# RazonIn4K/image-restoration-platform

Hardware: AMD Instinct MI355X
Metric: restored images/sec @1024x1024 bs=8 (higher is better)
Workload: dtype bf16; 1 GPU; 1024x1024 RGB u8, batch 8 per GPU: fused classifier scan + RestoreNet-v0 (43 convs, 779.9 GFLOP/image), seeded random-init weights; global_batch=8, parallelism=per-image data parallel x1, no collective, streams=1

## Files before the change

image_restoration_platform_amd/csrc/conv_down.hip:

```cpp
#include "conv_mfma.hpp"
#include "persist.hpp"

namespace ire {

namespace {

typedef __bf16 bf16x8_t __attribute__((ext_vector_type(8)));
typedef __bf16 bf16x2_t __attribute__((ext_vector_type(2)));
typedef float f32x2_t __attribute__((ext_vector_type(2)));
typedef float f32x16_t __attribute__((ext_vector_type(16)));
typedef unsigned u32x4_t __attribute__((ext_vector_type(4)));

#ifndef DN_LD_NT
#define DN_LD_NT 0
#endif
constexpr int DN_THREADS = 512;
constexpr int DN_TH = 16, DN_TW = 32;
constexpr int DN_IH = DN_TH + 1, DN_IW = DN_TW + 1;
constexpr int DN_IN_CHUNKS = DN_IH * DN_IW * 4;
constexpr int DN_IN_ITERS = (DN_IN_CHUNKS + DN_THREADS - 1) / DN_THREADS;
constexpr int DN_IN_BYTES = DN_IN_ITERS * DN_THREADS * 16;
constexpr int DN_NT = 64, DN_NTL = 2;
constexpr int DN_W_BYTES_MAX = 4 * 4 * DN_NT * 16;
constexpr int DN_W_BASE = 2 * DN_IN_BYTES;
constexpr int DN_MAIN = DN_W_BASE + 3 * DN_W_BYTES_MAX;
constexpr int DN_RED_HALF = 8 * (DN_NT / 8) * 4 * 4;
constexpr int DN_LDS = DN_MAIN + 2 * DN_RED_HALF + 256 * 4;
static_assert(DN_LDS <= 160 * 1024, "LDS");

__device__ __forceinline__ unsigned dn_pack(float a, float b) {
    f32x2_t f = {a, b};
    return __builtin_bit_cast(unsigned, __builtin_convertvector(f, bf16x2_t));
}
__device__ __forceinline__ void dn_glds16(const void* gsrc, unsigned lds_dst_uniform) {
    unsigned keep;
    asm volatile("s_mov_b32 %0, m0\n\ts_mov_b32 m0, %2\n\ts_nop 0\n\tglobal_load_lds_dwordx4 %1, off\n\ts_mov_b32 m0, %0"
                 : "=&s"(keep) : "v"(gsrc), "s"(lds_dst_uniform) : "memory");
}
template <int N> __device__ __forceinline__ float dn_ror_add(float v) {
    const int r = __builtin_amdgcn_update_dpp(0, __builtin_bit_cast(int, v), 0x120 + N, 0xf, 0xf, false);
    return v + __builtin_bit_cast(float, r);
}
__device__ __forceinline__ float dn_swap16_add(float v) {
    float x = v, y = v;
    asm volatile("v_nop\n\tv_nop\n\tv_permlane16_swap_b32 %0, %1" : "+v"(x), "+v"(y));
    return x + y;
}

__host__ __device__ constexpr int dn_ntaps(int p) { return ((p >> 1) ? 2 : 1) * ((p & 1) ? 2 : 1); }
__host__ __device__ constexpr int dn_slab_off(int p) { return p == 0 ? 0 : p == 1 ? 4096 : p == 2 ? 12288 : 20480; }
constexpr int DN_GROUP_BYTES = 9 * 4 * DN_NT * 16;

struct DnRegs { u32x4_t v[DN_IN_ITERS]; };
__host__ __device__ constexpr int dn_dma_iters(int p) { return (dn_ntaps(p) * 4 * DN_NT + DN_THREADS - 1) / DN_THREADS; }
template <int N> __device__ __forceinline__ void dn_wait_vm(bool counted) {
    if (counted) asm volatile("s_waitcnt vmcnt(%0)" :: "n"(N) : "memory");
    else asm volatile("s_waitcnt vmcnt(0)" ::: "memory");
}

__global__ __launch_bounds__(DN_THREADS) void conv_down_kernel(ConvArgs a) {
    __shared__ __attribute__((aligned(16))) unsigned char smem[DN_LDS];
    const unsigned smem_lds = (unsigned)(size_t)(__attribute__((address_space(3))) unsigned char*)smem;
    const int tid = threadIdx.x;
    const int lane = tid & 63, wave = tid >> 6;
    const int r = lane & 31, h = lane >> 5;
    const int c8_fixed = tid & 3;

    const int tiles_per_img = a.tiles_x * a.tiles_y;
    const int nkc = a.nkc;
    PersistCursor cursor(a.tiles_x, a.tiles_y, a.nimg, a.nblocks, 4 * nkc, (int)gridDim.x, (int)blockIdx.x, a.walk_rev != 0);
    const int my_items = cursor.my_items;
    const int S = cursor.S;
    if (S == 0) return;
    using StageInfo = PersistStage;
    StageInfo sq0 = cursor.cur, sq1 = cursor.next(), sq2 = cursor.next();

    const int Cin = a.cin0;
    const int cin_shift = 31 - __builtin_clz(Cin);

    int a_off[2][4];
#pragma unroll
    for (int m = 0; m < 2; ++m)
#pragma unroll
        for (int o = 0; o < 4; ++o) {
            const int dy = (o >> 1) - 1, dx = (o & 1) - 1;
            const int p = (wave * 2 + m + 1 + dy) * DN_IW + r + 1 + dx;
            a_off[m][o] = (p * 4 + (h ^ ((p >> 2) & 3))) * 16;
        }
    const int b_off = (h * DN_NT + r) * 16;

    unsigned coff[DN_IN_ITERS], cokb = 0;
    auto item_offsets = [&](const PersistItem& it) {
        const int y0 = 2 * (it.ty * DN_TH - 1), x0 = 2 * (it.tx * DN_TW - 1);
        int t2 = tid;
// ... 66 lines not shown
            const int gg = (st_nb * DN_NT) / Gs + tid;
            float* st = a.stats + (((size_t)st_img * tiles_per_img + st_tile) * 8 + gg) * 2;
            st[0] = s; st[1] = q;
        }
        st_img = -1;
    };
    auto init_acc = [&](int nb) {
        const float* bl = bias_lds + nb * DN_NT + 8 * h;
#pragma unroll
        for (int j = 0; j < DN_NTL; ++j)
#pragma unroll
            for (int q = 0; q < 4; ++q) {
                const float4 bv = *reinterpret_cast<const float4*>(bl + j * 32 + 16 * (q >> 1) + 4 * (q & 1));
#pragma unroll
                for (int m = 0; m < 2; ++m) { acc[m][j][4 * q + 0] = bv.x; acc[m][j][4 * q + 1] = bv.y; acc[m][j][4 * q + 2] = bv.z; acc[m][j][4 * q + 3] = bv.w; }
            }
    };
    auto epilogue = [&](const PersistItem& it) __attribute__((always_inline)) {
        int r_e = r, h_e = h, w_e = wave;
        asm volatile("" : "+v"(r_e), "+v"(h_e), "+v"(w_e));
        char* obase = reinterpret_cast<char*>(a.out) + (size_t)it.img * a.Hout * a.Wout * a.cout * 2;
        const __amdgpu_buffer_rsrc_t orsrc = __builtin_amdgcn_make_buffer_rsrc(obase, 0, a.Hout * a.Wout * a.cout * 2, 0x00020000);
        const bf16x2_t ones = __builtin_bit_cast(bf16x2_t, 0x3f803f80u);
        float* redw = red_base + red_par * (DN_RED_HALF / 4);
        const int ox = it.tx * DN_TW + r_e;
        bool inb[2];
        unsigned offs[2];
#pragma unroll
        for (int m = 0; m < 2; ++m) {
            const int oy = it.ty * DN_TH + w_e * 2 + m;
            inb[m] = oy < a.Hout && ox < a.Wout;
            offs[m] = ((unsigned)((oy * a.Wout + ox) * a.cout + it.nb * DN_NT) << 1) + (unsigned)(h_e * 16);
        }
#pragma unroll
        for (int j = 0; j < DN_NTL; ++j)
#pragma unroll
            for (int pp = 0; pp < 2; ++pp) {
                float sA = 0.f, qA = 0.f;
#pragma unroll
                for (int m = 0; m < 2; ++m) {
                    const f32x16_t& c = acc[m][j];
                    const unsigned w[4] = {dn_pack(c[8 * pp + 0], c[8 * pp + 1]), dn_pack(c[8 * pp + 2], c[8 * pp + 3]),
                                           dn_pack(c[8 * pp + 4], c[8 * pp + 5]), dn_pack(c[8 * pp + 6], c[8 * pp + 7])};
                    float ts = 0.f, tq = 0.f;
#pragma unroll
                    for (int d = 0; d < 4; ++d) {
                        const bf16x2_t wv = __builtin_bit_cast(bf16x2_t, w[d]);
                        ts = __builtin_amdgcn_fdot2_f32_bf16(wv, ones, ts, false);
                        tq = __builtin_amdgcn_fdot2_f32_bf16(wv, wv, tq, false);
                    }
                    sA += inb[m] ? ts : 0.f; qA += inb[m] ? tq : 0.f;
                    const u32x4_t wv4 = {w[0], w[1], w[2], w[3]};
                    __builtin_amdgcn_raw_buffer_store_b128(wv4, orsrc, inb[m] ? offs[m] + (unsigned)(j * 64 + pp * 32) : 0xffffffffu, 0, IRE_ST_PART);
                }
                sA = dn_ror_add<1>(sA); qA = dn_ror_add<1>(qA);
                sA = dn_ror_add<2>(sA); qA = dn_ror_add<2>(qA);
                sA = dn_ror_add<4>(sA); qA = dn_ror_add<4>(qA);
                sA = dn_ror_add<8>(sA); qA = dn_ror_add<8>(qA);
                sA = dn_swap16_add(sA); qA = dn_swap16_add(qA);
                if ((lane & 31) == 0) {
                    float* d = redw + (wave * 8 + j * 4 + 2 * pp + h_e) * 4;
                    d[0] = sA; d[1] = qA; d[2] = 0.f; d[3] = 0.f;
                }
            }
#pragma unroll
        for (int m = 0; m < 2; ++m)
#pragma unroll
            for (int j = 0; j < DN_NTL; ++j) asm volatile("" : "=v"(acc[m][j]));
        st_img = it.img; st_tile = it.tile; st_nb = it.nb; st_par = red_par; red_par ^= 1;
    };

    DnRegs R0, R1;
    int widx = 0;
    bool warm = false;
    auto stage = [&](auto phase_tag, auto last_tag) {
        constexpr int PHASE = decltype(phase_tag)::value, PAR = PHASE & 1;
        constexpr bool LAST = decltype(last_tag)::value;
        constexpr int PA = PHASE >> 1, PB = PHASE & 1, NTY = PA ? 2 : 1, NTX = PB ? 2 : 1, NTAPS = NTY * NTX;
        constexpr int D1 = dn_dma_iters((PHASE + 1) & 3), D2 = dn_dma_iters((PHASE + 2) & 3);
        const unsigned char* ib = smem + PAR * DN_IN_BYTES;
        uint4* in_nxt = reinterpret_cast<uint4*>(smem + (PAR ^ 1) * DN_IN_BYTES);
        const unsigned char* wb = smem + DN_W_BASE + widx * DN_W_BYTES_MAX + b_off;
        const int w2 = widx == 0 ? 2 : widx - 1;
        DnRegs& Rn = PAR ? R0 : R1;
        DnRegs& Rf = PAR ? R1 : R0;
        load_stage(sq2, Rf);
        {
            constexpr int NPH = (PHASE + 2) & 3;
            constexpr int pieces = dn_ntaps(NPH) * 4 * DN_NT;
            const unsigned char* ws = wslab(sq2);
            const int wave_u = __builtin_amdgcn_readfirstlane(wave);
            const unsigned w_dst_lds = smem_lds + (unsigned)(DN_W_BASE + w2 * DN_W_BYTES_MAX);
#pragma unroll
            for (int i = 0; i < D2; ++i) {
                int cbase = i * DN_THREADS + wave_u * 64;
                if ((i + 1) * DN_THREADS > pieces) cbase = cbase % pieces;
                dn_glds16(ws + (size_t)(cbase + lane) * 16, w_dst_lds + cbase * 16);
// ... 47 lines not shown
        for (int i = 0; i < DN_IN_ITERS; ++i) asm volatile("" : "+v"(R0.v[i]));
        const uint4* ws0 = reinterpret_cast<const uint4*>(wslab(sq0));
        const uint4* ws1 = reinterpret_cast<const uint4*>(wslab(sq1));
        uint4* wd = reinterpret_cast<uint4*>(smem + DN_W_BASE);
        for (int i = tid; i < dn_ntaps(0) * 4 * DN_NT; i += DN_THREADS) wd[i] = ws0[i];
        for (int i = tid; i < dn_ntaps(1) * 4 * DN_NT; i += DN_THREADS) wd[DN_W_BYTES_MAX / 16 + i] = ws1[i];
        uint4* in0 = reinterpret_cast<uint4*>(smem);
#pragma unroll
        for (int i = 0; i < DN_IN_ITERS; ++i) store_chunk(i, R0, in0);
        load_stage(sq1, R1);
    }
    __syncthreads();
    for (int k = 0; k < my_items; ++k) {
        init_acc(sq0.it.nb);
        for (int kc = 0; kc + 1 < nkc; ++kc) {
            stage(std::integral_constant<int, 0>{}, std::false_type{}); stage(std::integral_constant<int, 1>{}, std::false_type{});
            stage(std::integral_constant<int, 2>{}, std::false_type{}); stage(std::integral_constant<int, 3>{}, std::false_type{});
        }
        stage(std::integral_constant<int, 0>{}, std::false_type{}); stage(std::integral_constant<int, 1>{}, std::false_type{});
        stage(std::integral_constant<int, 2>{}, std::false_type{}); stage(std::integral_constant<int, 3>{}, std::true_type{});
    }
    asm volatile("s_waitcnt vmcnt(0)" ::: "memory");
    __syncthreads();
    flush_stats();
}

}

void conv_down_launch(const ConvArgs& a, hipStream_t stream) {
    if (a.cout % 64 || a.cout > 256 || a.nkc < 1 || a.stats == nullptr) fail(IRE_ERR_INTERNAL, "internal: conv_down shape");
    const int items = a.tiles_x * a.tiles_y * a.nimg * a.nblocks;
    const int cus = persistent_grid_cus();
    const int grid = items < cus ? items : cus;
    hipLaunchKernelGGL(conv_down_kernel, dim3(grid), dim3(DN_THREADS), 0, stream, a);
    IRE_HIP(hipGetLastError());
}

}
```

image_restoration_platform_amd/csrc/conv_mfma.hpp:

```cpp
#pragma once
#include "common.hpp"
#include "conv_kind.hpp"

#ifndef IRE_ST_LINE
#define IRE_ST_LINE 16
#endif
#ifndef IRE_LD_ONCE
#define IRE_LD_ONCE 2
#endif
#ifndef IRE_LD_IN
#define IRE_LD_IN 0
#endif
#ifndef IRE_ST_PART
#define IRE_ST_PART 0
#endif

#include <cstdlib>

namespace ire {

inline int persistent_grid_cus() {
    static const int forced = [] { const char* v = std::getenv("IRE_GRID_CUS"); return v ? std::atoi(v) : 0; }();
    int dev = 0, cus = 256;
    (void)hipGetDevice(&dev);
// ... 7 lines not shown
    const void* in0;
    const void* in1;
    int cin0, cin1;
    int kc_split;
    int nkc;
    const unsigned short* w;
    const unsigned short* w1;
    const float* bias;
    const float2* ab;
    const float* gn_stats;
    int gn_parts, gn_hw;
    const float* gn_gamma;
    const float* gn_beta;
    const float* gn_film;
    int gn_film_stride, gn_film_off;
    float2* ab_w;
    const unsigned short* resid;
    unsigned short* out;
    const unsigned char* u8_in;
    unsigned char* u8_out;
    float* stats;
    int Hin, Win, Hout, Wout, cout;
    int tiles_x, tiles_y, nimg, nblocks;
    int group_size;
    int prio_young;
    int in_rows;
    int in_row_off;
    int iy_lo, iy_span;
    int fp8;
    const float* oscale;
    int w4_nt;
    const void* zeros;
    unsigned long long* stamps;
    int walk_rev;
};

void conv_launch(ConvKind kind, const ConvArgs& a, hipStream_t stream);

void conv_rb_launch(bool resid, bool fused_act, const ConvArgs& a, hipStream_t stream);
void conv_w4_launch(bool resid, const ConvArgs& a, hipStream_t stream);
void conv_f8_launch(bool resid, const ConvArgs& a, hipStream_t stream);
void conv_stem_launch(const ConvArgs& a, hipStream_t stream);
void conv_down_launch(const ConvArgs& a, hipStream_t stream);
void conv_head_launch(const ConvArgs& a, hipStream_t stream);
void conv_pc_launch(bool resid, bool head, const ConvArgs& a, hipStream_t stream);
void conv_pk_launch(bool resid, const ConvArgs& a, hipStream_t stream);
void conv_up_subpixel_launch(const ConvArgs& a, hipStream_t stream);
void conv_upq_launch(const ConvArgs& a, hipStream_t stream);
void conv_dnq_launch(const ConvArgs& a, hipStream_t stream);
void conv_up_launch(const ConvArgs& a, hipStream_t stream);

}
```

image_restoration_platform_amd/csrc/conv_stem.hip:

```cpp
#include "conv_mfma.hpp"
#include "persist.hpp"

#include <type_traits>

namespace ire {

namespace {

typedef __bf16 bf16x8_t __attribute__((ext_vector_type(8)));
typedef __bf16 bf16x2_t __attribute__((ext_vector_type(2)));
typedef float f32x2_t __attribute__((ext_vector_type(2)));
typedef float f32x16_t __attribute__((ext_vector_type(16)));
typedef unsigned u32x4_t __attribute__((ext_vector_type(4)));

constexpr int ST_THREADS = 512, ST_TH = 16, ST_TW = 32, ST_IH = ST_TH + 2, ST_IW = ST_TW + 2;
constexpr int ST_RB = ST_IW * 3;
constexpr int ST_PW = ST_IW + 2;
constexpr int ST_ROW = ST_PW * 4;
constexpr int ST_ITERS = (ST_IH * ST_RB + ST_THREADS - 1) / ST_THREADS;

__device__ __forceinline__ unsigned st_pack(float a, float b) {
    f32x2_t f = {a, b};
    return __builtin_bit_cast(unsigned, __builtin_convertvector(f, bf16x2_t));
}
template <int N> __device__ __forceinline__ float st_ror_add(float v) {
    const int r = __builtin_amdgcn_update_dpp(0, __builtin_bit_cast(int, v), 0x120 + N, 0xf, 0xf, false);
    return v + __builtin_bit_cast(float, r);
}
__device__ __forceinline__ float st_swap16_add(float v) {
    float x = v, y = v;
    asm volatile("v_nop\n\tv_nop\n\tv_permlane16_swap_b32 %0, %1" : "+v"(x), "+v"(y));
    return x + y;
}

__global__ __launch_bounds__(ST_THREADS) void conv_stem_kernel(ConvArgs a) {
    __shared__ __attribute__((aligned(16))) unsigned short tile[2][ST_IH * ST_ROW];
    __shared__ float red[2][8][8][2];
    const int tid = threadIdx.x, lane = tid & 63, wave = tid >> 6, r = lane & 31, h = lane >> 5;

    const u32x4_t* wf = reinterpret_cast<const u32x4_t*>(a.w);
    const bf16x8_t w0 = __builtin_bit_cast(bf16x8_t, wf[(0 * 2 + h) * 32 + r]);
    const bf16x8_t w1 = __builtin_bit_cast(bf16x8_t, wf[(1 * 2 + h) * 32 + r]);
    const bf16x8_t w2 = __builtin_bit_cast(bf16x8_t, wf[(2 * 2 + h) * 32 + r]);
    f32x16_t bias_acc;
#pragma unroll
    for (int i = 0; i < 16; ++i) bias_acc[i] = a.bias[16 * (i >> 3) + 8 * h + (i & 7)];
    const int foff = (2 * wave * ST_PW + r + 2 * h) * 4;
    for (int i = tid; i < 2 * ST_IH * ST_ROW / 2; i += ST_THREADS) reinterpret_cast<unsigned*>(&tile[0][0])[i] = 0u;
    __syncthreads();
    int spy[ST_ITERS], sb[ST_ITERS], spx[ST_ITERS], srel[ST_ITERS];
#pragma unroll
    for (int it = 0; it < ST_ITERS; ++it) {
        const int i = tid + it * ST_THREADS;
        spy[it] = i / ST_RB; sb[it] = i - spy[it] * ST_RB;
        spx[it] = sb[it] / 3;
        srel[it] = (spy[it] * a.Win + spx[it]) * 3 + (sb[it] - spx[it] * 3);
    }

    const int tiles_per_img = a.tiles_x * a.tiles_y;
    const unsigned char* in = reinterpret_cast<const unsigned char*>(a.in0);
    const bf16x2_t ones = __builtin_bit_cast(bf16x2_t, 0x3f803f80u);
    unsigned pv[ST_ITERS];
    auto request = [&](const PersistItem& ri) {
        const int iy0 = ri.ty * ST_TH - 1, ix0 = ri.tx * ST_TW - 1;
        const long long base = (((long long)ri.img * a.in_rows + iy0 + a.in_row_off) * a.Win + ix0) * 3;
#pragma unroll
        for (int it = 0; it < ST_ITERS; ++it) {
            const bool ok = spy[it] < ST_IH && (unsigned)(iy0 + spy[it] - a.iy_lo) < (unsigned)a.iy_span && (unsigned)(ix0 + spx[it]) < (unsigned)a.Win;
            const unsigned v = in[ok ? base + srel[it] : 0];
            pv[it] = ok ? v : 0u;
        }
    };
    int par = 0;
    PersistCursor cursor(a.tiles_x, a.tiles_y, a.nimg, 1, 1, (int)gridDim.x, (int)blockIdx.x, a.walk_rev != 0);
    const int n_items = cursor.my_items;
    PersistItem nx = cursor.cur.it;
    if (n_items > 0) request(nx);
    for (int k = 0; k < n_items; ++k) {
        const int img = nx.img, t = nx.tile, ty = nx.ty, tx = nx.tx;
        unsigned short* tl = tile[par];
#pragma unroll
        for (int it = 0; it < ST_ITERS; ++it)
            if (spy[it] < ST_IH) tl[spy[it] * ST_ROW + spx[it] * 4 + (sb[it] - spx[it] * 3)] = (unsigned short)(__builtin_bit_cast(unsigned, (float)pv[it]) >> 16);
        if (k + 1 < n_items) { nx = cursor.next().it; request(nx); }
        __syncthreads();
        const int ox = tx * ST_TW + r;
        char* obase = reinterpret_cast<char*>(a.out) + (size_t)img * a.Hout * a.Wout * 64;
        float gs[2][2] = {{0.f, 0.f}, {0.f, 0.f}}, gq[2][2] = {{0.f, 0.f}, {0.f, 0.f}};
#pragma unroll
        for (int m = 0; m < 2; ++m) {
            u32x4_t f[3];
#pragma unroll
            for (int ky = 0; ky < 3; ++ky) {
                const uint2* fp = reinterpret_cast<const uint2*>(tl + foff + (m + ky) * ST_ROW);
                const uint2 lo = fp[0], hi = fp[1];
                f[ky] = u32x4_t{lo.x, lo.y, hi.x, hi.y};
            }
            f32x16_t c = __builtin_amdgcn_mfma_f32_32x32x16_bf16(w0, __builtin_bit_cast(bf16x8_t, f[0]), bias_acc, 0, 0, 0);
            c = __builtin_amdgcn_mfma_f32_32x32x16_bf16(w1, __builtin_bit_cast(bf16x8_t, f[1]), c, 0, 0, 0);
            c = __builtin_amdgcn_mfma_f32_32x32x16_bf16(w2, __builtin_bit_cast(bf16x8_t, f[2]), c, 0, 0, 0);
            const int oy = ty * ST_TH + 2 * wave + m;
            const bool inb = ox < a.Wout && oy < a.Hout;
            const float mf = inb ? 1.f : 0.f;
#pragma unroll
            for (int pp = 0; pp < 2; ++pp) {
                const unsigned w[4] = {st_pack(c[8 * pp + 0], c[8 * pp + 1]), st_pack(c[8 * pp + 2], c[8 * pp + 3]),
                                       st_pack(c[8 * pp + 4], c[8 * pp + 5]), st_pack(c[8 * pp + 6], c[8 * pp + 7])};
#pragma unroll
                for (int d = 0; d < 4; ++d) {
                    const bf16x2_t wv = __builtin_bit_cast(bf16x2_t, w[d]);
                    const float s1 = __builtin_amdgcn_fdot2_f32_bf16(wv, ones, 0.f, false), q1 = __builtin_amdgcn_fdot2_f32_bf16(wv, wv, 0.f, false);
                    gs[pp][d >> 1] = __builtin_fmaf(s1, mf, gs[pp][d >> 1]);
                    gq[pp][d >> 1] = __builtin_fmaf(q1, mf, gq[pp][d >> 1]);
                }
                if (inb) {
                    const u32x4_t wv4 = {w[0], w[1], w[2], w[3]};
                    *reinterpret_cast<u32x4_t*>(obase + ((size_t)oy * a.Wout + ox) * 64 + (16 * pp + 8 * h) * 2) = wv4;
                }
            }
            __builtin_amdgcn_sched_barrier(0);
        }
        if (a.stats) {
            const bool b0 = lane & 1, b1 = lane & 2;
            auto xch = [&](float keep, float give, auto ctrl_tag) __attribute__((always_inline)) -> float {
                const int gg = __builtin_amdgcn_update_dpp(0, __builtin_bit_cast(int, give), decltype(ctrl_tag)::value, 0xf, 0xf, false);
                return keep + __builtin_bit_cast(float, gg);
            };
            const float vs[4] = {gs[0][0], gs[0][1], gs[1][0], gs[1][1]}, vq[4] = {gq[0][0], gq[0][1], gq[1][0], gq[1][1]};
            float u[4], t2[2];
#pragma unroll
            for (int k = 0; k < 4; ++k) u[k] = xch(b0 ? vq[k] : vs[k], b0 ? vs[k] : vq[k], std::integral_constant<int, 0xb1>{});
#pragma unroll
            for (int k = 0; k < 2; ++k) t2[k] = xch(b1 ? u[2 + k] : u[k], b1 ? u[k] : u[2 + k], std::integral_constant<int, 0x4e>{});
            t2[0] = st_ror_add<4>(t2[0]); t2[1] = st_ror_add<4>(t2[1]);
            t2[0] = st_ror_add<8>(t2[0]); t2[1] = st_ror_add<8>(t2[1]);
            t2[0] = st_swap16_add(t2[0]); t2[1] = st_swap16_add(t2[1]);
            if ((lane & 28) == 0) {
                const int g0 = 4 * (b1 ? 1 : 0) + 2 * h;
                red[par][wave][g0][b0 ? 1 : 0] = t2[0];
                red[par][wave][g0 + 1][b0 ? 1 : 0] = t2[1];
            }
            __syncthreads();
            if (tid < 8) {
                float s = 0.f, q = 0.f;
#pragma unroll
                for (int w = 0; w < 8; ++w) { s += red[par][w][tid][0]; q += red[par][w][tid][1]; }
                float* st = a.stats + (((size_t)img * tiles_per_img + t) * 8 + tid) * 2;
                st[0] = s; st[1] = q;
            }
        }
        par ^= 1;
    }
}

}

void conv_stem_launch(const ConvArgs& a, hipStream_t stream) {
    if (a.cout != 32 || a.Hout != a.Hin || a.Wout != a.Win || !a.stats) fail(IRE_ERR_INTERNAL, "internal: conv_stem shape");
    const int items = a.tiles_x * a.tiles_y * a.nimg;
    const int cus = persistent_grid_cus();
    const int grid = items < 2 * cus ? items : 2 * cus;
    hipLaunchKernelGGL(conv_stem_kernel, dim3(grid), dim3(ST_THREADS), 0, stream, a);
    IRE_HIP(hipGetLastError());
}

}
```

image_restoration_platform_amd/csrc/engine.cpp:

```cpp
#include "engine.hpp"
#include "encode.hpp"
#include "deflate.hpp"
#include "jpeg.hpp"
#include "jpeg_dec.hpp"

#include <chrono>
#include <cmath>
#include <cstdlib>
#include <cstring>
#include <fstream>

#include "gn.hpp"
#include "strips.hpp"
#include "weight_pack.hpp"
#include "grey_tables.inc"

namespace ire {

namespace {

inline double now_s() {
    return std::chrono::duration<double>(std::chrono::steady_clock::now().time_since_epoch()).count();
}

}

Engine::Engine(const ire_config& cfg) {
    int ndev = 0;
    hipError_t e = hipGetDeviceCount(&ndev);
    if (e != hipSuccess || ndev <= 0)
        fail(IRE_ERR_UNAVAILABLE, "service unavailable: no HIP device visible (the engine has no CPU fallback)");
    device_ = cfg.device_index;
    if (device_ < 0 || device_ >= ndev) fail(IRE_ERR_INVALID_INPUT, "invalid device_index");
    IRE_HIP(hipSetDevice(device_));
    hipDeviceProp_t prop;
    IRE_HIP(hipGetDeviceProperties(&prop, device_));
    if (std::strncmp(prop.gcnArchName, "gfx950", 6) != 0)
        fail(IRE_ERR_UNAVAILABLE, std::string("service unavailable: device is ") + prop.gcnArchName +
                                      ", this engine is built for gfx950 (MI355X) only");
    if (cfg.precision != IRE_PRECISION_BF16 && cfg.precision != IRE_PRECISION_FP8) fail(IRE_ERR_INVALID_INPUT, "invalid precision");
    precision_ = cfg.precision;
    max_batch_ = cfg.max_batch > 0 ? cfg.max_batch : 8;
    if (max_batch_ > 64) fail(IRE_ERR_INVALID_INPUT, "invalid max_batch (1..64)");
    num_lanes_ = cfg.num_streams > 0 ? cfg.num_streams : 1;
    if (num_lanes_ > 16) num_lanes_ = 16;
    constexpr uint32_t kResultBits = IRE_FLAG_RESULT_PNG_BASE64 | IRE_FLAG_RESULT_PNG_DEFLATE | IRE_FLAG_RESULT_JPEG;
    if (cfg.flags & ~(kResultBits | IRE_FLAG_DECODE_PROGRESSIVE)) fail(IRE_ERR_INVALID_INPUT, "invalid ire_config.flags (unknown bits set)");
    if (((cfg.flags & kResultBits) & ((cfg.flags & kResultBits) - 1)) != 0) fail(IRE_ERR_INVALID_INPUT, "invalid ire_config.flags (two result formats set)");
    flags_ = cfg.flags;
    sw_ = ConvSwitches::from_env();
    cus_ = persistent_grid_cus();
    if (const char* v = std::getenv("IRE_SNAKE")) snake_ = std::atoi(v) != 0;
    if (const char* v = std::getenv("IRE_JPEG_DEC_TIMES")) dec_times_ = std::atoi(v) != 0;
    if (const char* v = std::getenv("IRE_JPEG_DEC_WINDOWS")) dec_min_windows_ = (uint32_t)std::max(0, std::atoi(v));
    if (const char* v = std::getenv("IRE_RB_STAMPS")) {
        stamps_cout_ = std::atoi(v);
        stamps_resid_ = std::strchr(v, 'r') != nullptr;
    }
    if (const char* v = std::getenv("IRE_W4_TL")) stamps_tl_ = v;

    IRE_HIP(hipStreamCreateWithFlags(&main_stream_, hipStreamNonBlocking));
    for (auto& ev : ev_) IRE_HIP(hipEventCreate(&ev));
    IRE_HIP(hipEventCreateWithFlags(&fork_ev_, hipEventDisableTiming));
    IRE_HIP(hipEventCreateWithFlags(&busy_ev_, hipEventDisableTiming));
    lanes_.resize(num_lanes_);
    for (auto& L : lanes_) {
        IRE_HIP(hipStreamCreateWithFlags(&L.stream, hipStreamNonBlocking));
        IRE_HIP(hipEventCreateWithFlags(&L.done, hipEventDisableTiming));
    }

    unsigned int* d_lin = tables_mem_.alloc<unsigned int>(sizeof(kLin16));
    unsigned int* d_thr = tables_mem_.alloc<unsigned int>(sizeof(kGreyThr));
    unsigned char* d_inv = tables_mem_.alloc<unsigned char>(5008);
    IRE_HIP(hipMemset(d_inv, 0, 5008));
    IRE_HIP(hipMemcpy(d_lin, kLin16, sizeof(kLin16), hipMemcpyHostToDevice));
    IRE_HIP(hipMemcpy(d_thr, kGreyThr, sizeof(kGreyThr), hipMemcpyHostToDevice));
    IRE_HIP(hipMemcpy(d_inv, kGreyInv, sizeof(kGreyInv), hipMemcpyHostToDevice));
    tables_ = ClassifierTables{d_lin, d_thr, d_inv};
    if (stamps_cout_) {
        stamps_dev_.grow(8 * 2 * 64 * 10 * 8);
        IRE_HIP(hipMemset(stamps_dev_.get<void>(), 0, 8 * 2 * 64 * 10 * 8));
    }

    if (cfg.weights_path && cfg.weights_path[0]) load_weights_file(cfg.weights_path);
}
// ... 636 lines not shown
    const ConvDesc& d = cw.desc;
    ConvSite site;
    site.lin = op.lin; site.lout = op.lout; site.use_ab = op.use_ab; site.has_in1 = op.in1 != BUF_NONE; site.stats_out = op.stats_out;
    site.nimg = g.nimg; site.h = g.h; site.w = g.w; site.H = g.H; site.halo = g.halo; site.has_up = g.has_up; site.has_down = g.has_down;
    site.y0 = g.y0; site.cus = cus_;
    const ConvPlan p = plan_conv(sw_, d, site, precision_ == IRE_PRECISION_FP8);

    auto in_ptr = [&](int id) -> const unsigned short* { return id == BUF_NONE ? nullptr : g.buf[id >> 3][id & 7]; };
    auto out_ptr = [&](int id) -> unsigned short* {
        if (id == BUF_NONE) return nullptr;
        const int l = id >> 3;
        return g.buf[l][id & 7] + (size_t)g.halo * (g.w >> l) * kWidths[l];
    };
    const int Hout = g.h >> op.lout, Wout = g.w >> op.lout;
    ConvArgs a{};
    a.in0 = (d.kind == CONV_STEM) ? (const void*)g.img_in : (const void*)in_ptr(op.in0);
    a.in1 = in_ptr(op.in1);
    if (p.in1_first_row) a.in1 = in_ptr(op.in1) + (size_t)g.halo * Wout * d.cout;
    a.cin0 = d.cin0; a.cin1 = p.cin1; a.kc_split = d.kc_split; a.nkc = p.nkc; a.nblocks = p.nblocks; a.w4_nt = p.w4_nt; a.fp8 = p.fp8;
    const unsigned short* const slabs[] = {nullptr, cw.d_w, cw.d_wp, cw.d_w4, cw.d_w4h, cw.d_wstem, cw.d_wd, cw.d_wu, cw.d_wuf, cw.d_wdq, cw.d_wuq, cw.d_wsq,
                                           cw.d_wsk, reinterpret_cast<const unsigned short*>(cw.d_w8x), reinterpret_cast<const unsigned short*>(cw.d_w8)};
    const float* const biases[] = {cw.d_bias, cw.d_bias_uf, cw.d_bias8};
    a.w = slabs[p.w]; a.w1 = slabs[p.w1]; a.bias = biases[p.bias];
    if (p.fp8) a.oscale = cw.d_oscale;
    if (p.zeros) a.zeros = d_zero_.get<void>();
    a.ab = op.use_ab ? R.ab : nullptr; a.resid = out_ptr(op.resid); a.out = out_ptr(op.out);
    a.u8_in = d.kind == CONV_HEAD ? g.img_in + (size_t)g.halo * g.w * 3 : nullptr;
    a.u8_out = d.kind == CONV_HEAD ? g.img_out : nullptr;
    a.Hin = g.h >> op.lin; a.Win = g.w >> op.lin; a.Hout = Hout; a.Wout = Wout;
    a.in_rows = p.in_rows; a.in_row_off = p.in_row_off; a.iy_lo = p.iy_lo; a.iy_span = p.iy_span;
    a.cout = p.cout; a.group_size = p.group_size; a.tiles_x = p.tiles_x; a.tiles_y = p.tiles_y; a.nimg = g.nimg;
    if (op.stats_out) a.stats = (R.stats_alt ? R.stats_alt : R.stats) + p.stats_offset();
    a.prio_young = sw_.prio_young;
    a.walk_rev = R.snake && R.next_rev && p.kernel != K_V1;
    R.next_rev = !a.walk_rev;
    const bool rb = d.kind == CONV_RB1 || d.kind == CONV_RB2;
    if (stamps_dev_ && rb && d.cout == stamps_cout_ && (d.kind == CONV_RB2) == stamps_resid_ && (!stamps_taken_ || !stamps_tl_.empty() || std::getenv("IRE_STAMPS_RAW"))) {
        a.stamps = stamps_dev_.get<unsigned long long>();
        stamps_taken_ = true;
    }
    if (R.gn_pending) {
        if (p.folds_gn) {
            const GNW& gn = *R.gn_pending;
            a.gn_stats = R.gn_stats; a.gn_parts = R.gn_parts; a.gn_hw = (g.H >> gn.level) * (g.w >> gn.level);
            a.gn_gamma = gn.d_gamma; a.gn_beta = gn.d_beta; a.gn_film = R.film; a.gn_film_stride = kFilmDim; a.gn_film_off = kFilmOff[gn.level];
            a.ab_w = R.ab;
            R.gn_pending = nullptr;
        } else flush_gn(R, g);
    }
    prof_begin(p.fam, R.stream, p.flops, p.bytes);
    switch (p.kernel) {
        case K_V1: conv_launch(d.kind, a, R.stream); break;
        case K_F8: conv_f8_launch(p.resid, a, R.stream); break;
        case K_PK: conv_pk_launch(p.resid, a, R.stream); break;
        case K_W4: conv_w4_launch(p.resid, a, R.stream); break;
        case K_PC: conv_pc_launch(p.resid, false, a, R.stream); break;
        case K_RB: conv_rb_launch(p.resid, p.fused_act, a, R.stream); break;
        case K_PC_HEAD: conv_pc_launch(false, true, a, R.stream); break;
        case K_RB_HEAD: conv_head_launch(a, R.stream); break;
        case K_DNQ: conv_dnq_launch(a, R.stream); break;
        case K_DOWN: conv_down_launch(a, R.stream); break;
        case K_STEM: conv_stem_launch(a, R.stream); break;
        case K_UPQ: conv_upq_launch(a, R.stream); break;
        case K_UP_FUSED:
        case K_UP_SUB: conv_up_subpixel_launch(a, R.stream); break;
        case K_UP_RB: conv_up_launch(a, R.stream); break;
    }
    prof_tag(p.key, p.kname, op.lout, d.cin, d.cout, p.flops_exec);
    prof_end(R.stream);
    if (op.stats_out) {
        R.stat_parts = p.stat_parts;
        if (R.stats_alt) std::swap(R.stats, R.stats_alt);
    }
    if (capture_ && !op.name.empty() && a.out && g.halo == 0) capture(op.name.c_str(), a.out, (size_t)g.nimg * Hout * Wout * d.cout, R.stream);
    if (capture_ && !op.name.empty() && a.out && g.halo == 1)
        capture_rows(op.name.c_str(), a.out, (size_t)Hout * Wout * d.cout, (size_t)(g.H >> op.lout) * Wout * d.cout,
                     (size_t)(g.y0 >> op.lout) * Wout * d.cout, R.stream);
    if (capture_ && a.ab != nullptr && g.halo == 0)
        capture_f32(((op.name.empty() ? std::string("head") : op.name) + ".ab").c_str(), reinterpret_cast<const float*>(R.ab), (size_t)g.nimg * d.cin * 2, R.stream);
}

void Engine::flush_gn(Run& R, const Geo& g) {
    const GNW& gn = *R.gn_pending;
    prof_begin(FAM_GN, R.stream, 0, 0);
    gn_finalize_launch(R.gn_stats, g.nimg, R.gn_parts, gn.C, (g.H >> gn.level) * (g.w >> gn.level), gn.d_gamma, gn.d_beta, R.film, kFilmDim,
                       kFilmOff[gn.level], R.ab, R.stream);
    prof_end(R.stream);
    R.gn_pending = nullptr;
}

void Engine::exec_op(Run& R, const Op& op, const Geo& g) {
    switch (op.kind) {
        case Op::GN: {
            R.gn_pending = op.gn; R.gn_stats = R.stats; R.gn_parts = R.stat_parts;
            if (!sw_.gn_fold || g.halo) flush_gn(R, g);
            break;
        }
        case Op::CONV: exec_conv(R, op, g); break;
    }
}

void Engine::run_network(Lane& L, int nimg, int h, int w, const uint8_t* d_in, uint8_t* d_out, const float* d_film) {
    Run R;
    R.stream = L.stream; R.stats = L.v.stats; R.stats_alt = L.v.stats2; R.ab = L.v.ab; R.film = d_film;
    R.snake = snake_;
    const Geo g = geo_of_lane(L, nimg, h, w, d_in, d_out);
    prof_chain_ = false;
    prof_chainable_ = capture_ == false;
    prof_skip_ = prof_on_ == 2 && prof_every_ > 1 && (prof_pass_ % prof_every_) != 0;
    ++prof_pass_;
// ... 229 lines not shown
```

image_restoration_platform_amd/csrc/engine.hpp:

```cpp
#pragma once
#include <deque>
#include <map>
#include <memory>
#include <mutex>
#include <string>
#include <vector>

#include "classifier.hpp"
#include "common.hpp"
#include "conv_mfma.hpp"
#include "conv_plan.hpp"
#include "device_buf.hpp"
#include "jpeg_dec.hpp"

namespace ire {

struct PackedConv;
struct ConvW {
    ConvDesc desc;
    unsigned short* d_w = nullptr;
    unsigned short* d_wp = nullptr;
    unsigned short* d_w4 = nullptr;
    unsigned short* d_w4h = nullptr;
    unsigned short* d_wstem = nullptr;
// ... 179 lines not shown
    void encode_host_impl(const uint8_t* rgb, int n, int h, int w, uint8_t* chars, size_t stride);
    void ensure_enc_scratch(size_t need, size_t full);
    uint8_t* ensure_enc_io(size_t need);
    void encode_deflate_window(const uint8_t* d_rgb, int n, int h, int w, size_t row_pitch, size_t image_pitch, uint8_t* d_chars, size_t stride, uint8_t* d_lens,
                               size_t lens_pitch, hipStream_t s);
    void encode_jpeg_window(const uint8_t* d_rgb, int n, int h, int w, size_t row_pitch, size_t image_pitch, uint8_t* d_chars, size_t stride, uint8_t* d_lens,
                            size_t lens_pitch, hipStream_t s);
    void encode_result(const uint8_t* d_rgb, int n, int h, int w, size_t row_pitch, size_t image_pitch, uint8_t* d_txt, size_t txt_stride, hipStream_t s);
    void ensure_io(int n, int h, int w);
    void ensure_workspace(int n, int h, int w);
    void free_workspace();
    void build_program();
    void run_network(Lane& L, int nimg, int h, int w, const uint8_t* d_in, uint8_t* d_out, const float* d_film);
    void exec_op(Run& R, const Op& op, const Geo& g);
    void flush_gn(Run& R, const Geo& g);
    void exec_conv(Run& R, const Op& op, const Geo& g);
    static Geo geo_of_lane(const Lane& L, int nimg, int h, int w, const uint8_t* d_in, uint8_t* d_out);
    void prof_begin(int fam, hipStream_t s, double flops, double bytes);
    void prof_tag(const char* key, const char* kernel, int level, int cin, int cout, double flops_exec);
    void prof_end(hipStream_t s);
    void capture(const char* name, const unsigned short* d, size_t count, hipStream_t s);
    void capture_rows(const char* name, const unsigned short* d, size_t count, size_t total, size_t offset, hipStream_t s);
    void capture_f32(const char* name, const float* d, size_t count, hipStream_t s);
    template <class T> T* upload(const std::vector<T>& v);
    ConvW upload_conv(const PackedConv& p);

    int device_ = 0;
    int max_batch_ = 8;
    int num_lanes_ = 1;
    uint32_t flags_ = 0;
    int precision_ = IRE_PRECISION_BF16;
    ConvSwitches sw_;
    int cus_ = 256;
    bool snake_ = true;
    std::mutex mu_;
    hipStream_t main_stream_ = nullptr;
    hipEvent_t ev_[4] = {};
    hipEvent_t fork_ev_ = nullptr;
    hipEvent_t busy_ev_ = nullptr;
    bool busy_recorded_ = false;
    int64_t batches_run_ = 0, images_restored_ = 0;
    int last_batch_ = 0;
    std::deque<std::pair<double, int>> recent_;
    double t0_ = 0.0;

    ClassifierTables tables_{};
    BufSet<DeviceMem> tables_mem_;

    IoBufs<DeviceMem> io_;
    int last_n_ = 0;
    FuseBufs<DeviceMem> fuse_;
    Buf<DeviceMem> d_zero_;
    Buf<DeviceMem> d_pp_tab_, d_pp_mid_, d_pp_in_, d_pp_out_;
    Buf<DeviceMem> d_enc_scratch_;
    Buf<DeviceMem> d_pad_in_, d_pad_out_;
    Buf<DeviceMem> d_enc_io_;
    struct DecScratch {
        Buf<PinnedMem> pin[2];
        Buf<DeviceMem> d_in, d_coef, d_planes;
        Buf<DeviceMem> d_lanes;
        Buf<DeviceMem> d_walk;
        hipEvent_t up_ev[2] = {};
        bool up_recorded[2] = {};
        int turn = 0;
        DecScratch() = default;
        DecScratch(const DecScratch&) = delete;
// ... 49 lines not shown
```

Before: 1058 images/sec.

## Transpose conv epilogue stores through LDS patches and vectorize stem input loads

Stem and down-conv epilogues now stage each wave's packed bf16 outputs in a swizzled LDS patch, then re-read them so lanes write full contiguous pixel rows with 16-byte stores. The aim is fewer partial, scattered global write transactions. The stem also loads its u8 input as aligned dwords per thread instead of per-byte gathers, with a slow path at row edges. Both paths are on by default via new engine flags. The cost is extra LDS, wave barriers and more register pressure.

```diff
diff --git a/image_restoration_platform_amd/csrc/conv_down.hip b/image_restoration_platform_amd/csrc/conv_down.hip
--- a/image_restoration_platform_amd/csrc/conv_down.hip
+++ b/image_restoration_platform_amd/csrc/conv_down.hip
@@ -13,6 +13,9 @@
 
 #ifndef DN_LD_NT
 #define DN_LD_NT 0
+#endif
+#ifndef DN_TEPI_ST
+#define DN_TEPI_ST IRE_ST_LINE
 #endif
 constexpr int DN_THREADS = 512;
 constexpr int DN_TH = 16, DN_TW = 32;
@@ -26,7 +29,8 @@
 constexpr int DN_MAIN = DN_W_BASE + 3 * DN_W_BYTES_MAX;
 constexpr int DN_RED_HALF = 8 * (DN_NT / 8) * 4 * 4;
 constexpr int DN_LDS = DN_MAIN + 2 * DN_RED_HALF + 256 * 4;
-static_assert(DN_LDS <= 160 * 1024, "LDS");
+constexpr int DN_PATCH_BYTES = 16 * DN_NT * 2;
+static_assert(DN_LDS + 8 * DN_PATCH_BYTES <= 160 * 1024, "LDS");
 
 __device__ __forceinline__ unsigned dn_pack(float a, float b) {
     f32x2_t f = {a, b};
@@ -58,8 +62,9 @@
     else asm volatile("s_waitcnt vmcnt(0)" ::: "memory");
 }
 
+template <bool TEPI>
 __global__ __launch_bounds__(DN_THREADS) void conv_down_kernel(ConvArgs a) {
-    __shared__ __attribute__((aligned(16))) unsigned char smem[DN_LDS];
+    __shared__ __attribute__((aligned(16))) unsigned char smem[DN_LDS + (TEPI ? 8 * DN_PATCH_BYTES : 0)];
     const unsigned smem_lds = (unsigned)(size_t)(__attribute__((address_space(3))) unsigned char*)smem;
     const int tid = threadIdx.x;
     const int lane = tid & 63, wave = tid >> 6;
@@ -192,6 +197,7 @@
             inb[m] = oy < a.Hout && ox < a.Wout;
             offs[m] = ((unsigned)((oy * a.Wout + ox) * a.cout + it.nb * DN_NT) << 1) + (unsigned)(h_e * 16);
         }
+        u32x4_t pkd[2][TEPI ? 2 * DN_NTL : 1];
 #pragma unroll
         for (int j = 0; j < DN_NTL; ++j)
 #pragma unroll
@@ -211,7 +217,8 @@
                     }
                     sA += inb[m] ? ts : 0.f; qA += inb[m] ? tq : 0.f;
                     const u32x4_t wv4 = {w[0], w[1], w[2], w[3]};
-                    __builtin_amdgcn_raw_buffer_store_b128(wv4, orsrc, inb[m] ? offs[m] + (unsigned)(j * 64 + pp * 32) : 0xffffffffu, 0, IRE_ST_PART);
+                    if constexpr (TEPI) pkd[m][2 * j + pp] = wv4;
+                    else __builtin_amdgcn_raw_buffer_store_b128(wv4, orsrc, inb[m] ? offs[m] + (unsigned)(j * 64 + pp * 32) : 0xffffffffu, 0, IRE_ST_PART);
                 }
                 sA = dn_ror_add<1>(sA); qA = dn_ror_add<1>(qA);
                 sA = dn_ror_add<2>(sA); qA = dn_ror_add<2>(qA);
@@ -223,6 +230,30 @@
                     d[0] = sA; d[1] = qA; d[2] = 0.f; d[3] = 0.f;
                 }
             }
+        if constexpr (TEPI) {
+            unsigned char* patch = smem + DN_LDS + w_e * DN_PATCH_BYTES;
+            const int p16 = r_e & 15, pq = lane >> 3, cq = lane & 7;
+#pragma unroll
+            for (int m = 0; m < 2; ++m) {
+                const int oy = it.ty * DN_TH + w_e * 2 + m;
+#pragma unroll
+                for (int q = 0; q < 2; ++q) {
+                    if ((r_e >> 4) == q) {
+#pragma unroll
+                        for (int g = 0; g < 2 * DN_NTL; ++g) *reinterpret_cast<u32x4_t*>(patch + p16 * 128 + (((2 * g + h_e) ^ (p16 & 7)) << 4)) = pkd[m][g];
+                    }
+                    __builtin_amdgcn_wave_barrier();
+#pragma unroll
+                    for (int k = 0; k < 2; ++k) {
+                        const int p = pq + 8 * k, px = it.tx * DN_TW + 16 * q + p;
+                        const u32x4_t v = *reinterpret_cast<const u32x4_t*>(patch + p * 128 + ((cq ^ (p & 7)) << 4));
+                        const unsigned off = ((unsigned)((oy * a.Wout + px) * a.cout + it.nb * DN_NT) << 1) + (unsigned)(cq * 16);
+                        __builtin_amdgcn_raw_buffer_store_b128(v, orsrc, oy < a.Hout && px < a.Wout ? off : 0xffffffffu, 0, DN_TEPI_ST);
+                    }
+                    __builtin_amdgcn_wave_barrier();
+                }
+            }
+        }
 #pragma unroll
         for (int m = 0; m < 2; ++m)
 #pragma unroll
@@ -336,7 +367,8 @@
     const int items = a.tiles_x * a.tiles_y * a.nimg * a.nblocks;
     const int cus = persistent_grid_cus();
     const int grid = items < cus ? items : cus;
-    hipLaunchKernelGGL(conv_down_kernel, dim3(grid), dim3(DN_THREADS), 0, stream, a);
+    if (a.down_tepi) hipLaunchKernelGGL(conv_down_kernel<true>, dim3(grid), dim3(DN_THREADS), 0, stream, a);
+    else hipLaunchKernelGGL(conv_down_kernel<false>, dim3(grid), dim3(DN_THREADS), 0, stream, a);
     IRE_HIP(hipGetLastError());
 }
 
diff --git a/image_restoration_platform_amd/csrc/conv_mfma.hpp b/image_restoration_platform_amd/csrc/conv_mfma.hpp
--- a/image_restoration_platform_amd/csrc/conv_mfma.hpp
+++ b/image_restoration_platform_amd/csrc/conv_mfma.hpp
@@ -63,6 +63,7 @@
     int w4_nt;
     const void* zeros;
     unsigned long long* stamps;
+    int stem_tepi, down_tepi;
     int walk_rev;
 };
 
diff --git a/image_restoration_platform_amd/csrc/conv_stem.hip b/image_restoration_platform_amd/csrc/conv_stem.hip
--- a/image_restoration_platform_amd/csrc/conv_stem.hip
+++ b/image_restoration_platform_amd/csrc/conv_stem.hip
@@ -13,11 +13,17 @@
 typedef float f32x16_t __attribute__((ext_vector_type(16)));
 typedef unsigned u32x4_t __attribute__((ext_vector_type(4)));
 
+#ifndef ST_TEPI_SC1
+#define ST_TEPI_SC1 0
+#endif
 constexpr int ST_THREADS = 512, ST_TH = 16, ST_TW = 32, ST_IH = ST_TH + 2, ST_IW = ST_TW + 2;
 constexpr int ST_RB = ST_IW * 3;
 constexpr int ST_PW = ST_IW + 2;
 constexpr int ST_ROW = ST_PW * 4;
 constexpr int ST_ITERS = (ST_IH * ST_RB + ST_THREADS - 1) / ST_THREADS;
+constexpr int ST_RD = (ST_RB + 3 + 3) / 4;
+static_assert(ST_IH * ST_RD <= ST_THREADS, "one dword per thread and tile");
+constexpr int ST_PATCH = ST_TW * 64;
 
 __device__ __forceinline__ unsigned st_pack(float a, float b) {
     f32x2_t f = {a, b};
@@ -33,9 +39,11 @@
     return x + y;
 }
 
+template <bool TEPI>
 __global__ __launch_bounds__(ST_THREADS) void conv_stem_kernel(ConvArgs a) {
     __shared__ __attribute__((aligned(16))) unsigned short tile[2][ST_IH * ST_ROW];
     __shared__ float red[2][8][8][2];
+    __shared__ __attribute__((aligned(16))) unsigned char patches[TEPI ? 8 * ST_PATCH : 16];
     const int tid = threadIdx.x, lane = tid & 63, wave = tid >> 6, r = lane & 31, h = lane >> 5;
 
     const u32x4_t* wf = reinterpret_cast<const u32x4_t*>(a.w);
@@ -59,33 +67,92 @@
 
     const int tiles_per_img = a.tiles_x * a.tiles_y;
     const unsigned char* in = reinterpret_cast<const unsigned char*>(a.in0);
+    if constexpr (TEPI) __builtin_amdgcn_s_waitcnt(0x0f70);
     const bf16x2_t ones = __builtin_bit_cast(bf16x2_t, 0x3f803f80u);
     unsigned pv[ST_ITERS];
-    auto request = [&](const PersistItem& ri) {
+    const int dpy = tid / ST_RD, dj = tid - dpy * ST_RD;
+    unsigned dv = 0u, db[4] = {0u, 0u, 0u, 0u}, dbok = 0u;
+    int dmis = 0;
+    bool dfast = false, dslow = false;
+    auto request = [&](const PersistItem& ri, auto first_tag) {
         const int iy0 = ri.ty * ST_TH - 1, ix0 = ri.tx * ST_TW - 1;
-        const long long base = (((long long)ri.img * a.in_rows + iy0 + a.in_row_off) * a.Win + ix0) * 3;
-#pragma unroll
-        for (int it = 0; it < ST_ITERS; ++it) {
-            const bool ok = spy[it] < ST_IH && (unsigned)(iy0 + spy[it] - a.iy_lo) < (unsigned)a.iy_span && (unsigned)(ix0 + spx[it]) < (unsigned)a.Win;
-            const unsigned v = in[ok ? base + srel[it] : 0];
-            pv[it] = ok ? v : 0u;
+        if constexpr (TEPI) {
+            const long long row0 = ((long long)ri.img * a.in_rows + iy0 + dpy + a.in_row_off) * a.Win * 3, row1 = row0 + (long long)a.Win * 3;
+            const long long first = row0 + (long long)ix0 * 3;
+            dmis = (int)((reinterpret_cast<unsigned long long>(in) + (unsigned long long)first) & 3ull);
+            const long long d0 = first - dmis + 4 * dj;
+            const bool rowok = dpy < ST_IH && (unsigned)(iy0 + dpy - a.iy_lo) < (unsigned)a.iy_span;
+            const bool whole = d0 >= row0 && d0 + 4 <= row1;
+            dfast = rowok && whole; dslow = rowok && !whole;
+            dbok = 0u;
+            if constexpr (decltype(first_tag)::value) {
+                dv = dfast ? *reinterpret_cast<const unsigned*>(in + d0) : 0u;
+                if (dslow) {
+#pragma unroll
+                    for (int i = 0; i < 4; ++i) {
+                        const bool ok = d0 + i >= row0 && d0 + i < row1;
+                        db[i] = in[ok ? d0 + i : row0];
+                        dbok |= ok ? 1u << i : 0u;
+                    }
+                }
+            } else {
+                const unsigned char* fp = dfast ? in + d0 : reinterpret_cast<const unsigned char*>(reinterpret_cast<unsigned long long>(in) & ~3ull);
+                asm volatile("global_load_dword %0, %1, off" : "+v"(dv) : "v"(fp) : "memory");
+                if (dslow) {
+#pragma unroll
+                    for (int i = 0; i < 4; ++i) {
+                        const bool ok = d0 + i >= row0 && d0 + i < row1;
+                        const unsigned char* bp = in + (ok ? d0 + i : row0);
+                        asm volatile("global_load_ubyte %0, %1, off" : "+v"(db[i]) : "v"(bp) : "memory");
+                        dbok |= ok ? 1u << i : 0u;
+                    }
+                }
+            }
+        } else {
+            const long long base = (((long long)ri.img * a.in_rows + iy0 + a.in_row_off) * a.Win + ix0) * 3;
+#pragma unroll
+            for (int it = 0; it < ST_ITERS; ++it) {
+                const bool ok = spy[it] < ST_IH && (unsigned)(iy0 + spy[it] - a.iy_lo) < (unsigned)a.iy_span && (unsigned)(ix0 + spx[it]) < (unsigned)a.Win;
+                const unsigned v = in[ok ? base + srel[it] : 0];
+                pv[it] = ok ? v : 0u;
+            }
+        }
+    };
+    auto stage_tile = [&](unsigned short* tl) {
+        if constexpr (TEPI) {
+            asm volatile("s_waitcnt vmcnt(0)" ::: "memory");
+            asm volatile("" : "+v"(dv), "+v"(db[0]), "+v"(db[1]), "+v"(db[2]), "+v"(db[3]));
+            if (dpy < ST_IH) {
+#pragma unroll
+                for (int i = 0; i < 4; ++i) {
+                    const int b = 4 * dj - dmis + i;
+                    if ((unsigned)b < (unsigned)ST_RB) {
+                        const int px = (b * 171) >> 9;
+                        const unsigned v = dfast ? (dv >> (8 * i)) & 0xffu : (dbok >> i) & 1u ? db[i] : 0u;
+                        tl[dpy * ST_ROW + px * 4 + (b - px * 3)] = (unsigned short)(__builtin_bit_cast(unsigned, (float)v) >> 16);
+                    }
+                }
+            }
+        } else {
+#pragma unroll
+            for (int it = 0; it < ST_ITERS; ++it)
+                if (spy[it] < ST_IH) tl[spy[it] * ST_ROW + spx[it] * 4 + (sb[it] - spx[it] * 3)] = (unsigned short)(__builtin_bit_cast(unsigned, (float)pv[it]) >> 16);
         }
     };
     int par = 0;
     PersistCursor cursor(a.tiles_x, a.tiles_y, a.nimg, 1, 1, (int)gridDim.x, (int)blockIdx.x, a.walk_rev != 0);
     const int n_items = cursor.my_items;
     PersistItem nx = cursor.cur.it;
-    if (n_items > 0) request(nx);
+    if (n_items > 0) request(nx, std::true_type{});
     for (int k = 0; k < n_items; ++k) {
         const int img = nx.img, t = nx.tile, ty = nx.ty, tx = nx.tx;
         unsigned short* tl = tile[par];
-#pragma unroll
-        for (int it = 0; it < ST_ITERS; ++it)
-            if (spy[it] < ST_IH) tl[spy[it] * ST_ROW + spx[it] * 4 + (sb[it] - spx[it] * 3)] = (unsigned short)(__builtin_bit_cast(unsigned, (float)pv[it]) >> 16);
-        if (k + 1 < n_items) { nx = cursor.next().it; request(nx); }
+        stage_tile(tl);
+        if (k + 1 < n_items) { nx = cursor.next().it; request(nx, std::false_type{}); }
         __syncthreads();
         const int ox = tx * ST_TW + r;
         char* obase = reinterpret_cast<char*>(a.out) + (size_t)img * a.Hout * a.Wout * 64;
+        unsigned char* patch = patches + (TEPI ? wave * ST_PATCH : 0);
         float gs[2][2] = {{0.f, 0.f}, {0.f, 0.f}}, gq[2][2] = {{0.f, 0.f}, {0.f, 0.f}};
 #pragma unroll
         for (int m = 0; m < 2; ++m) {
@@ -113,10 +180,27 @@
                     gs[pp][d >> 1] = __builtin_fmaf(s1, mf, gs[pp][d >> 1]);
                     gq[pp][d >> 1] = __builtin_fmaf(q1, mf, gq[pp][d >> 1]);
                 }
-                if (inb) {
-                    const u32x4_t wv4 = {w[0], w[1], w[2], w[3]};
-                    *reinterpret_cast<u32x4_t*>(obase + ((size_t)oy * a.Wout + ox) * 64 + (16 * pp + 8 * h) * 2) = wv4;
-                }
+                const u32x4_t wv4 = {w[0], w[1], w[2], w[3]};
+                if constexpr (TEPI) *reinterpret_cast<u32x4_t*>(patch + r * 64 + (((2 * pp + h) ^ ((r >> 1) & 3)) << 4)) = wv4;
+                else if (inb) *reinterpret_cast<u32x4_t*>(obase + ((size_t)oy * a.Wout + ox) * 64 + (16 * pp + 8 * h) * 2) = wv4;
+            }
+            if constexpr (TEPI) {
+                __builtin_amdgcn_wave_barrier();
+                const int pq = lane >> 2, cq = lane & 3;
+#pragma unroll
+                for (int k2 = 0; k2 < 2; ++k2) {
+                    const int p = pq + 16 * k2, px = tx * ST_TW + p;
+                    const u32x4_t v = *reinterpret_cast<const u32x4_t*>(patch + p * 64 + ((cq ^ ((p >> 1) & 3)) << 4));
+                    if (oy < a.Hout && px < a.Wout) {
+                        char* op = obase + ((size_t)oy * a.Wout + px) * 64 + cq * 16;
+#if ST_TEPI_SC1
+                        asm volatile("global_store_dwordx4 %0, %1, off sc1" :: "v"(op), "v"(v) : "memory");
+#else
+                        *reinterpret_cast<u32x4_t*>(op) = v;
+#endif
+                    }
+                }
+                __builtin_amdgcn_wave_barrier();
             }
             __builtin_amdgcn_sched_barrier(0);
         }
@@ -160,7 +244,8 @@
     const int items = a.tiles_x * a.tiles_y * a.nimg;
     const int cus = persistent_grid_cus();
     const int grid = items < 2 * cus ? items : 2 * cus;
-    hipLaunchKernelGGL(conv_stem_kernel, dim3(grid), dim3(ST_THREADS), 0, stream, a);
+    if (a.stem_tepi) hipLaunchKernelGGL(conv_stem_kernel<true>, dim3(grid), dim3(ST_THREADS), 0, stream, a);
+    else hipLaunchKernelGGL(conv_stem_kernel<false>, dim3(grid), dim3(ST_THREADS), 0, stream, a);
     IRE_HIP(hipGetLastError());
 }
 
diff --git a/image_restoration_platform_amd/csrc/engine.cpp b/image_restoration_platform_amd/csrc/engine.cpp
--- a/image_restoration_platform_amd/csrc/engine.cpp
+++ b/image_restoration_platform_amd/csrc/engine.cpp
@@ -51,6 +51,8 @@
     sw_ = ConvSwitches::from_env();
     cus_ = persistent_grid_cus();
     if (const char* v = std::getenv("IRE_SNAKE")) snake_ = std::atoi(v) != 0;
+    if (const char* v = std::getenv("IRE_STEM_TEPI")) stem_tepi_ = std::atoi(v) != 0;
+    if (const char* v = std::getenv("IRE_DOWN_TEPI")) down_tepi_ = std::atoi(v) != 0;
     if (const char* v = std::getenv("IRE_JPEG_DEC_TIMES")) dec_times_ = std::atoi(v) != 0;
     if (const char* v = std::getenv("IRE_JPEG_DEC_WINDOWS")) dec_min_windows_ = (uint32_t)std::max(0, std::atoi(v));
     if (const char* v = std::getenv("IRE_RB_STAMPS")) {
@@ -753,6 +755,7 @@
     a.cout = p.cout; a.group_size = p.group_size; a.tiles_x = p.tiles_x; a.tiles_y = p.tiles_y; a.nimg = g.nimg;
     if (op.stats_out) a.stats = (R.stats_alt ? R.stats_alt : R.stats) + p.stats_offset();
     a.prio_young = sw_.prio_young;
+    a.stem_tepi = stem_tepi_; a.down_tepi = down_tepi_;
     a.walk_rev = R.snake && R.next_rev && p.kernel != K_V1;
     R.next_rev = !a.walk_rev;
     const bool rb = d.kind == CONV_RB1 || d.kind == CONV_RB2;
@@ -797,6 +800,8 @@
     if (capture_ && !op.name.empty() && a.out && g.halo == 1)
         capture_rows(op.name.c_str(), a.out, (size_t)Hout * Wout * d.cout, (size_t)(g.H >> op.lout) * Wout * d.cout,
                      (size_t)(g.y0 >> op.lout) * Wout * d.cout, R.stream);
+    if (capture_ && op.stats_out && !op.name.empty() && g.halo == 0)
+        capture_f32((op.name + ".stats").c_str(), a.stats, (size_t)g.nimg * p.stat_parts * 16, R.stream);
     if (capture_ && a.ab != nullptr && g.halo == 0)
         capture_f32(((op.name.empty() ? std::string("head") : op.name) + ".ab").c_str(), reinterpret_cast<const float*>(R.ab), (size_t)g.nimg * d.cin * 2, R.stream);
 }
diff --git a/image_restoration_platform_amd/csrc/engine.hpp b/image_restoration_platform_amd/csrc/engine.hpp
--- a/image_restoration_platform_amd/csrc/engine.hpp
+++ b/image_restoration_platform_amd/csrc/engine.hpp
@@ -235,6 +235,8 @@
     int precision_ = IRE_PRECISION_BF16;
     ConvSwitches sw_;
     int cus_ = 256;
+    bool stem_tepi_ = true;
+    bool down_tepi_ = true;
     bool snake_ = true;
     std::mutex mu_;
     hipStream_t main_stream_ = nullptr;
```

Result: no change. 1058 images/sec, median of 2 (+0.1%).
